# brown-palm/goal-force

Measured on AMD Instinct MI355X. Metric: frames_per_sec (81-frame video / (50-step denoise loop + VAE decode), Wan2.2-I2V-A14B 832x480x81f), higher is better.
Workload: dtype bf16

## Files before the change

### goal_force_amd/_lib.py

```python
from __future__ import annotations

import ctypes
import os
import threading

_HERE = os.path.dirname(os.path.abspath(__file__))
LIB_PATH = os.path.join(_HERE, "libgoalforce_hip.so")
LIB_PATH = os.environ.get("GOALFORCE_HIP_LIB", LIB_PATH)

SYMBOLS = (
    "gf_version", "gf_last_error", "gf_abi_version", "gf_set_option", "gf_get_option", "gf_reset_options",
    "gf_modulation", "gf_layernorm_modulate", "gf_rmsnorm_rope", "gf_gemm_bf16", "gf_flash_attn_fwd",
    "gf_patchify_im2col", "gf_unpatchify", "gf_cfg_euler_step", "gf_act", "gf_add_bf16",
    "gf_force_map",
    "gf_vae_prep_latent", "gf_vae_im2col", "gf_vae_finish_latent", "gf_vae_rmsnorm_silu", "gf_softmax_rows", "gf_rowmax_neg_bf16", "gf_transpose_pad",
    "gf_vae_tile_blend", "gf_vae_tile_finalize",
    "gf_quant_fp8_rowscale", "gf_cast_fp8", "gf_gemm_fp8", "gf_layernorm_modulate_fp8", "gf_modulate", "gf_gate_residual", "gf_rope_apply", "gf_linear_vt32_fp8",
    "gf_flash_attn_fwd_lse", "gf_flash_attn_bwd", "gf_flash_attn_bwd_workspace_bytes",
    "gf_layernorm_bwd", "gf_rmsnorm_rope_bwd", "gf_colsum", "gf_act_bwd", "gf_mse_loss", "gf_adamw_step", "gf_f32_to_bf16", "gf_sumsq",
    "gf_transpose_v", "gf_flash_attn_fwd_vt", "gf_transpose_v32", "gf_flash_attn_fwd_vt32", "gf_linear_vt32",
    "gf_conv3d_bf16", "gf_conv3d_padded_bf16", "gf_vae_rmsnorm_silu_padded", "gf_vae_upsample2x_padded", "gf_gemm_bf16_batched", "gf_transpose_pad_batched",
    "gf_resize_lanczos4_u8", "gf_resize_area_u8", "gf_canny_u8", "gf_flash_attn_fwd_lastmult",
)

ABI_VERSION = 18

EPI_BIAS, EPI_BIAS_GELU_TANH, EPI_BIAS_GATE_RESID, EPI_BIAS_RESID, EPI_BIAS_SILU, EPI_BIAS_MUL = range(6)


class GoalForceError(RuntimeError):
    """Raised when the HIP library is missing or a gf_* call returns an error."""


_lib = None
_lock = threading.Lock()

_vp, _i64, _f32, _int = ctypes.c_void_p, ctypes.c_int64, ctypes.c_float, ctypes.c_int


def _declare(lib):
    lib.gf_version.restype = ctypes.c_char_p
    lib.gf_version.argtypes = []
    lib.gf_last_error.restype = ctypes.c_char_p
    lib.gf_last_error.argtypes = []
    lib.gf_abi_version.restype = _int
    lib.gf_abi_version.argtypes = []
    lib.gf_set_option.restype = _int
    lib.gf_set_option.argtypes = [ctypes.c_char_p, _int]
    lib.gf_get_option.restype = _int
    lib.gf_get_option.argtypes = [ctypes.c_char_p, ctypes.POINTER(_int)]
    lib.gf_reset_options.restype = None
    lib.gf_reset_options.argtypes = []
    sigs = {
        "gf_layernorm_modulate": [_vp, _vp, _vp, _vp, _vp, _vp, _i64, _i64, _i64, _i64, _f32, _vp],
        "gf_modulation": [_vp, _vp, _vp, _i64, _i64, _i64, ctypes.c_uint32, _vp],
        "gf_rmsnorm_rope": [_vp, _vp, _vp, _vp, _i64, _i64, _i64, _i64, _f32, _vp],
        "gf_gemm_bf16": [_vp, _i64, _vp, _i64, _vp, _vp, _i64, _i64, _i64, _i64, _int, _vp, _i64, _vp, _vp],
        "gf_flash_attn_fwd": [_vp, _vp, _vp, _vp, _i64, _i64, _i64, _i64, _i64, _i64, _i64, _i64, _f32, _vp],
        "gf_flash_attn_fwd_lastmult": [_vp, _vp, _vp, _vp, _i64, _i64, _i64, _i64, _i64, _i64, _i64, _i64, _f32, _f32, _vp],
        "gf_flash_attn_fwd_lse": [_vp, _vp, _vp, _vp, _vp, _i64, _i64, _i64, _i64, _i64, _i64, _i64, _i64, _f32, _vp],
        "gf_flash_attn_bwd": [_vp] * 10 + [_i64] * 12 + [_f32, _vp],
        "gf_flash_attn_bwd_workspace_bytes": [_i64] * 3,
        "gf_layernorm_bwd": [_vp, _i64, _vp, _i64, _vp, _vp, _i64, _vp, _vp, _i64, _i64, _f32, _vp],
        "gf_rmsnorm_rope_bwd": [_vp, _i64, _vp, _i64, _vp, _vp, _vp, _vp, _i64, _vp, _i64, _i64, _i64, _f32, _vp],
        "gf_colsum": [_vp, _i64, _vp, _i64, _vp, _vp, _i64, _vp, _i64, _i64, _vp],
        "gf_act_bwd": [_vp, _vp, _vp, _i64, _int, _vp],
        "gf_mse_loss": [_vp, _vp, _vp, _vp, _i64, _f32, _vp],
        "gf_adamw_step": [_vp, _vp, _vp, _vp, _i64, _f32, _f32, _f32, _f32, _f32, _i64, _f32, _vp],
        "gf_f32_to_bf16": [_vp, _vp, _i64, _vp],
        "gf_sumsq": [_vp, _i64, _vp, _vp],
        "gf_transpose_v": [_vp, _i64, _vp, _i64, _i64, _i64, _vp],
        "gf_flash_attn_fwd_vt": [_vp, _vp, _vp, _vp, _vp, _i64, _i64, _i64, _i64, _i64, _i64, _i64, _i64, _f32, _vp],
        "gf_transpose_v32": [_vp, _i64, _vp, _i64, _i64, _i64, _vp],
        "gf_linear_vt32": [_vp, _i64, _vp, _i64, _vp, _vp, _i64, _i64, _i64, _i64, _vp],
        "gf_flash_attn_fwd_vt32": [_vp, _vp, _vp, _vp, _vp, _i64, _i64, _i64, _i64, _i64, _i64, _i64, _i64, _f32, _vp],
        "gf_patchify_im2col": [_vp, _i64, _vp, _i64, _vp, _i64, _i64, _i64, _i64, _vp],
        "gf_unpatchify": [_vp, _vp, _i64, _i64, _i64, _i64, _vp],
        "gf_cfg_euler_step": [_vp, _vp, _vp, _f32, _f32, _i64, _vp],
        "gf_act": [_vp, _vp, _i64, _int, _vp],
        "gf_add_bf16": [_vp, _vp, _vp, _i64, _vp],
        "gf_vae_prep_latent": [_vp, _i64, _i64, _i64, _i64, _vp, _vp, _vp, _i64, _i64, _i64, _i64, _i64, _vp],
        "gf_vae_im2col": [_vp, _vp, _vp, _i64, _i64, _i64, _i64, _i64, _i64, _int, _i64, _i64, _i64, _vp],
        "gf_conv3d_bf16": [_vp, _vp, _vp, _i64, _vp, _vp, _i64, _i64, _i64, _i64, _i64, _i64, _int, _int, _int, _int, _int,
                           _i64, _i64, _int, _vp, _i64, _vp],
        "gf_vae_finish_latent": [_vp, _i64, _vp, _vp, _vp, _i64, _i64, _vp],
        "gf_vae_rmsnorm_silu": [_vp, _vp, _vp, _i64, _i64, _int, _vp],
        "gf_vae_rmsnorm_silu_padded": [_vp, _vp, _vp, _i64, _i64, _i64, _i64, _int, _vp],
        "gf_conv3d_padded_bf16": [_vp, _vp, _i64, _vp, _vp, _i64, _i64, _i64, _i64, _i64, _i64, _i64, _int, _vp, _i64, _vp],
        "gf_vae_upsample2x_padded": [_vp, _vp, _i64, _i64, _i64, _i64, _vp],
        "gf_softmax_rows": [_vp, _i64, _vp, _i64, _vp, _i64, _i64, _i64, _i64, _f32, _vp],
        "gf_rowmax_neg_bf16": [_vp, _i64, _vp, _i64, _i64, _i64, _vp],
        "gf_transpose_pad": [_vp, _i64, _vp, _i64, _i64, _i64, _vp],
# ... 65 lines not shown
```

### goal_force_amd/csrc/gf_abi.hip

```cpp
#include "gf_common.h"
#include <cstdarg>
#include <cstdio>
#include <cstdlib>
#include <cstring>

#define GF_ABI_VERSION 18

static thread_local char g_err[512] = "";

void gf_set_error(const char* fmt, ...) {
    va_list ap;
    va_start(ap, fmt);
    vsnprintf(g_err, sizeof(g_err), fmt, ap);
    va_end(ap);
}

extern "C" GF_API const char* gf_version(void) { return "goalforce-hip 0.1.0 gfx950"; }
extern "C" GF_API const char* gf_last_error(void) { return g_err; }
extern "C" GF_API int gf_abi_version(void) { return GF_ABI_VERSION; }

static GfOptions g_options;

const GfOptions& gf_options() { return g_options; }

namespace {
struct OptionSlot {
    const char* name;
    std::atomic<int> GfOptions::*field;
    int lo, hi, dflt;
};
const OptionSlot kSlots[] = {
    {"prefer_8wave", &GfOptions::prefer_8wave, 0, 1, 0}, {"a4_stagger", &GfOptions::a4_stagger, 0, 1 << 20, 2},
    {"a4_group_m", &GfOptions::a4_group_m, 0, 64, 0},    {"conv_nb", &GfOptions::conv_nb, 0, 2, 0},
    {"conv_gather", &GfOptions::conv_gather, 0, 1, 0},   {"vae_rms3", &GfOptions::vae_rms3, 0, 1, 1},
    {"conv_direct", &GfOptions::conv_direct, 0, 1, 1},
};
}

extern "C" GF_API int gf_set_option(const char* name, int value) {
// ... 25 lines not shown
```

### goal_force_amd/dit.py

```python
from __future__ import annotations

import math
from typing import Optional, Tuple

import torch
import torch.nn as nn

from . import ops
from ._lib import GoalForceError


def precompute_freqs_cis(dim: int, end: int = 1024, theta: float = 10000.0):
    freqs = 1.0 / (theta ** (torch.arange(0, dim, 2)[: (dim // 2)].double() / dim))
    freqs = torch.outer(torch.arange(end), freqs)
    return torch.polar(torch.ones_like(freqs), freqs)


def precompute_freqs_cis_3d(dim: int, end: int = 1024, theta: float = 10000.0):
    return (precompute_freqs_cis(dim - 2 * (dim // 3), end, theta),
            precompute_freqs_cis(dim // 3, end, theta),
            precompute_freqs_cis(dim // 3, end, theta))


class RopeTable:
# ... 204 lines not shown
        x2 = _tokens2d(x)
        a = self.attend(x2, _as_rope(freqs, x.device))
        return linear(a, self.o).view(x.shape)


class CrossAttention(nn.Module):

    def __init__(self, dim: int, num_heads: int, eps: float = 1e-6, has_image_input: bool = False):
        super().__init__()
        if has_image_input:
            raise NotImplementedError("has_image_input=True (CLIP image tokens) is outside the Goal-Force path")
        self.dim, self.num_heads, self.head_dim = dim, num_heads, dim // num_heads
        self.q, self.k, self.v, self.o = (nn.Linear(dim, dim) for _ in range(4))
        self.norm_q, self.norm_k = RMSNorm(dim, eps=eps), RMSNorm(dim, eps=eps)
        self.has_image_input = False

    def context_kv(self, ctx2: torch.Tensor, fold: bool = True, pad_n: Optional[int] = None):
        m = 1
        if fold and ctx2.is_cuda and ops._OPT["fold_pad_keys"]:
            n = pad_run(ctx2) if pad_n is None else pad_n
            if ctx2.shape[0] - n >= 2 and n + 1 < ops.VT_MIN_KV:
                m = ctx2.shape[0] - n
                ctx2 = ctx2[: n + 1]
        cin = QuantizedInput(ctx2) if getattr(self.k, "_gf_w8", None) is not None else ctx2
        k, v = linear(cin, self.k), linear(cin, self.v)
        ops.rmsnorm_rope(k, self.norm_k.weight, None, None, self.head_dim, self.norm_k.eps)
        return k, v, m

    def attend(self, x2, kv):
        q = linear(x2, self.q)
        ops.rmsnorm_rope(q, self.norm_q.weight, None, None, self.head_dim, self.norm_q.eps)
        return ops.flash_attn(q, kv[0], kv[1], self.num_heads, last_key_mult=kv[2] if len(kv) > 2 else 1)

    def forward(self, x: torch.Tensor, y: torch.Tensor):
        x2 = _tokens2d(x)
        a = self.attend(x2, self.context_kv(_tokens2d(y)))
        return linear(a, self.o).view(x.shape)


class GateModule(nn.Module):

    def forward(self, x, gate, residual):
        if x.shape != residual.shape:
            raise GoalForceError("GateModule: x and residual must have the same shape")
        d = x.shape[-1]
        g = gate.reshape(-1, d)
        if x.dim() == 3 and g.shape[0] == x.shape[0] and x.shape[0] > 1:
            return torch.stack([ops.gate_residual(x[b], g[b].contiguous(), residual[b]) for b in range(x.shape[0])])
        if g.shape[0] != 1:
            raise GoalForceError("GateModule: gate must be [B or 1, 1, D] (per-token gates are outside the Goal-Force path)")
        return ops.gate_residual(x, g[0].contiguous(), residual)


class DiTBlock(nn.Module):

    def __init__(self, has_image_input: bool, dim: int, num_heads: int, ffn_dim: int, eps: float = 1e-6):
        super().__init__()
        self.dim, self.num_heads, self.ffn_dim, self.eps = dim, num_heads, ffn_dim, eps
        self.self_attn = SelfAttention(dim, num_heads, eps)
        self.cross_attn = CrossAttention(dim, num_heads, eps, has_image_input=has_image_input)
        self.norm1 = nn.LayerNorm(dim, eps=eps, elementwise_affine=False)
        self.norm2 = nn.LayerNorm(dim, eps=eps, elementwise_affine=False)
        self.norm3 = nn.LayerNorm(dim, eps=eps)
        self.ffn = nn.Sequential(nn.Linear(dim, ffn_dim), nn.GELU(approximate="tanh"), nn.Linear(ffn_dim, dim))
        self.modulation = nn.Parameter(torch.randn(1, 6, dim) / dim ** 0.5)
        self.gate = GateModule()
# ... 6 lines not shown
        rope = _as_rope(freqs, x.device)
        mod = ops.modulation(self.modulation, t_mod.contiguous(), onep_mask=0b010010)
        fp8 = getattr(self.ffn[0], "_gf_w8", None) is not None
        if self_attn_memo is not None and "x" in self_attn_memo:
            x_new = self_attn_memo.pop("x")
            ev = self_attn_memo.pop("ev", None)
            if ev is not None:
                torch.cuda.current_stream(x_new.device).wait_event(ev)
                x_new.record_stream(torch.cuda.current_stream(x_new.device))
            if out is not None:
                x_new = out.copy_(x_new)
            h = None if fp8 else torch.empty_like(x2)
        else:
            if fp8:
                h = QuantizedInput.layernorm(x2, scale1p=mod[1], shift=mod[0], eps=self.eps)
            else:
                h = ops.layernorm_modulate(x2, scale1p=mod[1], shift=mod[0], eps=self.eps)
            a = self.self_attn.attend(h, rope, sp, keep)
            x_new = out if out is not None else torch.empty_like(x2)
            linear(a, self.self_attn.o, epilogue=ops.EPI_BIAS_GATE_RESID, resid=x2, gate=mod[2], out=x_new)
            if keep is not None and keep.get("wide"):
                keep["x1"] = x_new.clone()
            if self_attn_memo is not None:
                self_attn_memo["x"] = x_new.clone()
                if x_new.is_cuda:
                    self_attn_memo["ev"] = torch.cuda.Event()
                    self_attn_memo["ev"].record(torch.cuda.current_stream(x_new.device))
        if fp8:
            h = QuantizedInput.layernorm(x_new, weight=self.norm3.weight, bias=self.norm3.bias, eps=self.eps)
        else:
            ops.layernorm_modulate(x_new, weight=self.norm3.weight, bias=self.norm3.bias, eps=self.eps, out=h)
        if context_kv is None:
            context_kv = self.cross_attn.context_kv(_tokens2d(context), fold=fold_pad_keys and keep is None, pad_n=pad_n)
        a = self.cross_attn.attend(h, context_kv)
        linear(a, self.cross_attn.o, epilogue=ops.EPI_BIAS_RESID, resid=x_new, out=x_new)
        if keep is not None and keep.get("wide"):
            keep["x2b"] = x_new.clone()
        if fp8:
            h = QuantizedInput.layernorm(x_new, scale1p=mod[4], shift=mod[3], eps=self.eps)
        else:
            ops.layernorm_modulate(x_new, scale1p=mod[4], shift=mod[3], eps=self.eps, out=h)
        f1 = linear(h, self.ffn[0], epilogue=ops.EPI_BIAS_GELU_TANH)
        linear(f1, self.ffn[2], epilogue=ops.EPI_BIAS_GATE_RESID, resid=x_new, gate=mod[5], out=x_new)
        return x_new.view(x.shape)


class Head(nn.Module):

    def __init__(self, dim: int, out_dim: int, patch_size: Tuple[int, int, int], eps: float):
        super().__init__()
        self.dim, self.patch_size, self.eps = dim, patch_size, eps
        self.norm = nn.LayerNorm(dim, eps=eps, elementwise_affine=False)
        self.head = nn.Linear(dim, out_dim * math.prod(patch_size))
        self.modulation = nn.Parameter(torch.randn(1, 2, dim) / dim ** 0.5)

    def forward(self, x, t_mod):
        if t_mod.dim() == 3:
            raise NotImplementedError("per-token head modulation is outside the Goal-Force path")
        x2 = _tokens2d(x)
        mod = ops.modulation(self.modulation, t_mod.contiguous(), onep_mask=0b10)
        h = ops.layernorm_modulate(x2, scale1p=mod[1], shift=mod[0], eps=self.eps)
        y = ops.gemm(h, self.head.weight, self.head.bias)
        return y.view(x.shape[:-1] + (y.shape[-1],))


class WanModel(nn.Module):

    def __init__(self, dim: int, in_dim: int, ffn_dim: int, out_dim: int, text_dim: int, freq_dim: int, eps: float,
# ... 101 lines not shown
```

### goal_force_amd/model_fn.py

```python
from __future__ import annotations

from typing import Optional

import torch

from . import ops
from ._lib import GoalForceError
from .dit import WanModel, pad_run


class ContextCache:

    def __init__(self):
        self.ctx = None
        self.pad_n = None
        self.dit_kv = {}
        self.cn_kv = {}


def _unsupported(name, value, default=None):
    if value is not None and value is not default and value is not False:
        raise NotImplementedError(f"model_fn_wan_video: `{name}` is outside the Goal-Force sampling path "
                                  "(SURVEY.md §2 #2)")


@torch.no_grad()
def model_fn_wan_video(
    dit: WanModel,
    motion_controller=None,
    vace=None,
    latents: torch.Tensor = None,
    timestep: torch.Tensor = None,
    context: torch.Tensor = None,
    clip_feature: Optional[torch.Tensor] = None,
    y: Optional[torch.Tensor] = None,
    reference_latents=None,
    vace_context=None,
    vace_scale=1.0,
    audio_embeds: Optional[torch.Tensor] = None,
    motion_latents: Optional[torch.Tensor] = None,
    s2v_pose_latents: Optional[torch.Tensor] = None,
    drop_motion_frames: bool = True,
    tea_cache=None,
    use_unified_sequence_parallel: bool = False,
    motion_bucket_id: Optional[torch.Tensor] = None,
    sliding_window_size: Optional[int] = None,
    sliding_window_stride: Optional[int] = None,
    cfg_merge: bool = False,
    use_gradient_checkpointing: bool = False,
    use_gradient_checkpointing_offload: bool = False,
# ... 29 lines not shown

    t, t_mod = dit.time_embed(timestep)

    if context_cache is not None and context_cache.ctx is not None:
        ctx, pad_n = context_cache.ctx, context_cache.pad_n
    else:
        ctx = dit.embed_text(context)
        pad_n = pad_run(ctx[0]) if ops._OPT["fold_pad_keys"] else None
        if context_cache is not None:
            context_cache.ctx, context_cache.pad_n = ctx, pad_n

    x, (f, h, w) = dit.patchify(latents, extra=y if (y is not None and dit.require_vae_embedding) else None)
    x = x[0]
    rope = dit.rope_table(f, h, w, latents.device)
    if sp is not None:
        x = sp.shard_tokens(x).contiguous()
        rope = dit.rope_table_shard(f, h, w, latents.device, sp)

    run_cn = use_controlnet and not (elide_zero_controlnet and controlnet.all_zero())
    c = None
    if run_cn:
        if controlnet.stride is not None:
            raise NotImplementedError("strided ControlNet (apply_strided_controlnet) is not used by Goal Force")
        control_latents = kwargs.get("control_signal_video_latents", None)
        if control_latents is None:
            raise GoalForceError("controlnet given but control_signal_video_latents missing")
        c = controlnet.controlnet_patch_embedding(control_latents)[0]
        if sp is not None:
            c = sp.shard_tokens(c).contiguous()
        n_cn = controlnet.controlnet_dit.num_layers
    else:
        n_cn = 0

    def kv_for(cache_dict, block, idx):
        if context_cache is None:
            return None
        if idx not in cache_dict:
            cache_dict[idx] = block.cross_attn.context_kv(ctx[0], pad_n=pad_n)
        return cache_dict[idx]

    for block_id, block in enumerate(dit.blocks):
        memo_cn = memo_dit = None
        if cfg_shared is not None and block_id == 0:
            memo_cn, memo_dit = cfg_shared.setdefault("cn0", {}), cfg_shared.setdefault("dit0", {})
        if block_id < n_cn:
            cb = controlnet.controlnet_dit.blocks[block_id]
            c = cb(c, ctx, t_mod, rope, context_kv=kv_for(context_cache.cn_kv if context_cache else None, cb, block_id),
                   sp=sp, self_attn_memo=memo_cn, pad_n=pad_n)
        x = block(x, ctx, t_mod, rope, context_kv=kv_for(context_cache.dit_kv if context_cache else None, block, block_id),
                  sp=sp, self_attn_memo=memo_dit, pad_n=pad_n)
        if block_id < n_cn:
            ops.gemm(c, controlnet.zero_conv_weight(block_id), controlnet.controlnet_zero_convs_after[block_id].bias,
                     epilogue=ops.EPI_BIAS_RESID, resid=x, out=x)

    x = dit.head(x.unsqueeze(0), t)
    if sp is not None:
        x = sp.gather_tokens(x[0], total=f * h * w).unsqueeze(0)
    return dit.unpatchify(x, (f, h, w))
```

### goal_force_amd/ops.py

```python
from __future__ import annotations

import math

import torch

from . import _lib
from ._lib import (EPI_BIAS, EPI_BIAS_GATE_RESID, EPI_BIAS_GELU_TANH, EPI_BIAS_MUL, EPI_BIAS_RESID, EPI_BIAS_SILU,
                   GoalForceError)

__all__ = [
    "modulation", "layernorm_modulate", "rmsnorm_rope", "gate_residual", "gemm", "flash_attn", "patchify_im2col", "unpatchify",
    "cfg_euler_step", "act", "add", "force_map",
    "EPI_BIAS", "EPI_BIAS_GELU_TANH", "EPI_BIAS_GATE_RESID", "EPI_BIAS_RESID", "EPI_BIAS_SILU", "EPI_BIAS_MUL",
]

_BF16 = torch.bfloat16

PROFILE_ATTN = None
PROFILE_GEMM = None
PROFILE_CONV = None


def _stream(t: torch.Tensor):
    if t.device.index != torch.cuda.current_device():
# ... 123 lines not shown
        out = torch.empty(a.shape[:-1] + (N,), dtype=_BF16, device=a.device)
    ov, Mo, No, ldc = _rows2d(out, "gemm.out")
    if (Mo, No) != (M, N):
        raise GoalForceError(f"gemm.out: expected [{M}, {N}], got [{Mo}, {No}]")
    ldr = 0
    if resid is not None:
        _req(resid, "gemm.resid")
        rv, Mr, Nr, ldr = _rows2d(resid, "gemm.resid")
        if (Mr, Nr) != (M, N):
            raise GoalForceError("gemm.resid: shape mismatch")
        resid = rv
    if gate is not None:
        _req(gate, "gemm.gate")
        if gate.numel() != N or not gate.is_contiguous():
            raise GoalForceError(f"gemm.gate: expected contiguous [{N}]")
    if bias is not None:
        _req(bias, "gemm.bias")
        if bias.numel() != N or not bias.is_contiguous():
            raise GoalForceError(f"gemm.bias: expected contiguous [{N}]")
    prof = PROFILE_GEMM
    if prof is not None:
        e0, e1 = torch.cuda.Event(enable_timing=True), torch.cuda.Event(enable_timing=True)
        e0.record()
    _lib.check(_lib.load().gf_gemm_bf16(_ptr(av), lda, _ptr(w), w.stride(0), _ptr(bias), _ptr(ov), ldc, M, N, K,
                                        int(epilogue), _ptr(resid), ldr, _ptr(gate), _stream(a)), "gf_gemm_bf16")
    if prof is not None:
        e1.record()
        prof.append((e0, e1, M, N, K, int(epilogue)))
    return out


VT_MIN_KV = 2048
_LIB_DEFAULTS = {"prefer_8wave": 0, "a4_stagger": 2, "a4_group_m": 0, "conv_nb": 0, "conv_gather": 0, "conv_direct": 1, "vae_rms3": 1}
_OPT = {"attn_k3": True, "vt_from_gemm": True, "conv_padded": True, "fold_pad_keys": True, "attn_q_prescale": True, "vae_attn_offset": True}


def lib_option(name: str) -> int:
    import ctypes
    v = ctypes.c_int(0)
    _lib.check(_lib.load().gf_get_option(name.encode(), ctypes.byref(v)), f"gf_get_option({name})")
    return int(v.value)


class options:

    def __init__(self, **kv):
        for k in kv:
            if k not in _OPT and k not in _LIB_DEFAULTS:
                raise GoalForceError(f"ops.options: unknown option {k!r}")
        self.kv, self.old = kv, {}

    @staticmethod
    def _apply_one(k, v):
        if k in _OPT:
            _OPT[k] = bool(v)
        else:
            _lib.check(_lib.load().gf_set_option(k.encode(), int(v)), f"gf_set_option({k})")

    def __enter__(self):
        self.old = {}
        try:
            for k, v in self.kv.items():
                old = _OPT[k] if k in _OPT else lib_option(k)
                self._apply_one(k, v)
                self.old[k] = old
        except BaseException:
            self.__exit__(None, None, None)
# ... 83 lines not shown
    if prof is not None:
        e0, e1 = torch.cuda.Event(enable_timing=True), torch.cuda.Event(enable_timing=True)
        e0.record()
    lib = _lib.load()
    kv_pad = -(-skv // 64) * 64
    if last_key_mult != 1 and (vt is not None or skv >= VT_MIN_KV):
        raise GoalForceError("flash_attn: last_key_mult is for short key sequences (the text context), not the V^T path")
    if skv >= VT_MIN_KV and head_dim == 128 and num_heads * 128 * kv_pad < 2 ** 31:
        if finished_q and vt is not None:
            raise GoalForceError("flash_attn: finished_q goes to kernel 2, which does not take kernel 3's V^T operand")
        k3 = _OPT["attn_k3"] and not finished_q
        tr, fa = (lib.gf_transpose_v32, lib.gf_flash_attn_fwd_vt32) if k3 else (lib.gf_transpose_v, lib.gf_flash_attn_fwd_vt)
        if vt is None:
            vt = _vt_workspace(num_heads * 128 * kv_pad, q.device)
            _lib.check(tr(_ptr(v), v.stride(0), _ptr(vt), skv, kv_pad, num_heads, _stream(q)), "gf_transpose_v")
        elif vt.numel() < num_heads * 128 * kv_pad:
            raise GoalForceError("flash_attn.vt: buffer smaller than heads*128*kv_pad")
        _lib.check(fa(_ptr(q), _ptr(k), _ptr(vt), _ptr(out), None, sq, skv, kv_pad, num_heads, head_dim,
                      q.stride(0), k.stride(0), out.stride(0), float(scale), _stream(q)), "gf_flash_attn_fwd_vt")
    elif last_key_mult != 1:
        _lib.check(lib.gf_flash_attn_fwd_lastmult(_ptr(q), _ptr(k), _ptr(v), _ptr(out), sq, skv, num_heads, head_dim, q.stride(0),
                                                  k.stride(0), v.stride(0), out.stride(0), float(scale), float(last_key_mult), _stream(q)),
                   "gf_flash_attn_fwd_lastmult")
    else:
        _lib.check(lib.gf_flash_attn_fwd(_ptr(q), _ptr(k), _ptr(v), _ptr(out), sq, skv, num_heads, head_dim,
                                         q.stride(0), k.stride(0), v.stride(0), out.stride(0), float(scale),
                                         _stream(q)), "gf_flash_attn_fwd")
    if prof is not None:
        e1.record()
        prof.append((e0, e1, sq, skv, num_heads))
    return out


def flash_attn_lse(q, k, v, num_heads, scale=None):
    for n, t in (("q", q), ("k", k), ("v", v)):
        _req(t, f"flash_attn_lse.{n}")
        if t.dim() != 2 or t.stride(1) != 1:
            raise GoalForceError(f"flash_attn_lse.{n}: expected 2-D [len, heads*head_dim] with contiguous rows")
    sq, hd_all = q.shape
    skv = k.shape[0]
    head_dim = hd_all // num_heads
    if k.shape[1] != hd_all or v.shape != k.shape or head_dim * num_heads != hd_all:
        raise GoalForceError("flash_attn_lse: q/k/v shape mismatch")
    if scale is None:
        scale = 1.0 / math.sqrt(head_dim)
    out = torch.empty((sq, hd_all), dtype=_BF16, device=q.device)
    lse = torch.empty((sq, num_heads), dtype=torch.float32, device=q.device)
    lib = _lib.load()
    kv_pad = -(-skv // 64) * 64
    if skv >= VT_MIN_KV and head_dim == 128 and num_heads * 128 * kv_pad < 2 ** 31:
        vt = _vt_workspace(num_heads * 128 * kv_pad, q.device)
        k3 = _OPT["attn_k3"]
        tr, fa = (lib.gf_transpose_v32, lib.gf_flash_attn_fwd_vt32) if k3 else (lib.gf_transpose_v, lib.gf_flash_attn_fwd_vt)
        _lib.check(tr(_ptr(v), v.stride(0), _ptr(vt), skv, kv_pad, num_heads, _stream(q)), "gf_transpose_v")
        _lib.check(fa(_ptr(q), _ptr(k), _ptr(vt), _ptr(out), _ptr(lse), sq, skv, kv_pad, num_heads, head_dim,
                      q.stride(0), k.stride(0), out.stride(0), float(scale), _stream(q)), "gf_flash_attn_fwd_vt")
        return out, lse
    _lib.check(lib.gf_flash_attn_fwd_lse(_ptr(q), _ptr(k), _ptr(v), _ptr(out), _ptr(lse), sq, skv, num_heads, head_dim,
                                         q.stride(0), k.stride(0), v.stride(0), out.stride(0), float(scale),
                                         _stream(q)), "gf_flash_attn_fwd_lse")
    return out, lse


def flash_attn_bwd(q, k, v, o, dout, lse, num_heads, scale=None, need_dkv=True):
    for n, t in (("q", q), ("k", k), ("v", v), ("o", o), ("dout", dout)):
        _req(t, f"flash_attn_bwd.{n}")
# ... 552 lines not shown
```

### include/goalforce.h

```cpp
#ifndef GOALFORCE_H
#define GOALFORCE_H

#include <stdint.h>

#if defined(GF_BUILD)
#define GF_API __attribute__((visibility("default")))
#else
#define GF_API
#endif

#ifdef __cplusplus
extern "C" {
#endif

typedef enum {
    GF_OK = 0,
    GF_ERR_INVALID_ARG = -1,
    GF_ERR_UNSUPPORTED = -2,
    GF_ERR_LAUNCH = -3
} gf_status;

GF_API const char* gf_version(void);
GF_API const char* gf_last_error(void);
GF_API int gf_abi_version(void);
// ... 21 lines not shown
    GF_EPI_BIAS_SILU = 4,
    GF_EPI_BIAS_MUL = 5
} gf_epilogue;

GF_API int gf_gemm_bf16(const void* A, int64_t lda, const void* W, int64_t ldw, const void* bias,
                 void* C, int64_t ldc, int64_t M, int64_t N, int64_t K,
                 int epilogue, const void* resid, int64_t ldr, const void* gate,
                 void* stream);

GF_API int gf_gemm_bf16_batched(const void* A, int64_t lda, int64_t strideA, const void* W, int64_t ldw, int64_t strideW, void* C,
                                int64_t ldc, int64_t strideC, int64_t M, int64_t N, int64_t K, int64_t batch, void* stream);

GF_API int gf_flash_attn_fwd(const void* q, const void* k, const void* v, void* o,
                      int64_t q_len, int64_t kv_len, int64_t heads, int64_t head_dim,
                      int64_t q_stride, int64_t k_stride, int64_t v_stride, int64_t o_stride,
                      float scale, void* stream);

GF_API int gf_transpose_v(const void* v, int64_t v_stride, void* vt, int64_t kv_len, int64_t kv_pad, int64_t heads, void* stream);
GF_API int gf_flash_attn_fwd_vt(const void* q, const void* k, const void* vt, void* o, float* lse,
                         int64_t q_len, int64_t kv_len, int64_t kv_pad, int64_t heads, int64_t head_dim,
                         int64_t q_stride, int64_t k_stride, int64_t o_stride, float scale, void* stream);

GF_API int gf_transpose_v32(const void* v, int64_t v_stride, void* vt, int64_t kv_len, int64_t kv_pad, int64_t heads, void* stream);
GF_API int gf_flash_attn_fwd_vt32(const void* q, const void* k, const void* vt, void* o, float* lse,
                                  int64_t q_len, int64_t kv_len, int64_t kv_pad, int64_t heads, int64_t head_dim,
                                  int64_t q_stride, int64_t k_stride, int64_t o_stride, float scale, void* stream);

GF_API int gf_linear_vt32(const void* x, int64_t ldx, const void* w, int64_t ldw, const void* bias, void* vt,
                          int64_t kv_len, int64_t kv_pad, int64_t N, int64_t K, void* stream);

GF_API int gf_flash_attn_fwd_lastmult(const void* q, const void* k, const void* v, void* o, int64_t q_len, int64_t kv_len,
                                      int64_t heads, int64_t head_dim, int64_t q_stride, int64_t k_stride, int64_t v_stride,
                                      int64_t o_stride, float scale, float last_key_multiplicity, void* stream);

GF_API int gf_flash_attn_fwd_lse(const void* q, const void* k, const void* v, void* o, float* lse,
                          int64_t q_len, int64_t kv_len, int64_t heads, int64_t head_dim,
                          int64_t q_stride, int64_t k_stride, int64_t v_stride, int64_t o_stride,
                          float scale, void* stream);
GF_API int64_t gf_flash_attn_bwd_workspace_bytes(int64_t q_len, int64_t kv_len, int64_t heads);
GF_API int gf_flash_attn_bwd(const void* q, const void* k, const void* v, const void* o, const void* dout,
                      const float* lse, void* workspace, void* dq, void* dk, void* dv,
                      int64_t q_len, int64_t kv_len, int64_t heads, int64_t head_dim,
                      int64_t q_stride, int64_t k_stride, int64_t v_stride, int64_t o_stride, int64_t do_stride,
                      int64_t dq_stride, int64_t dk_stride, int64_t dv_stride, float scale, void* stream);

GF_API int gf_layernorm_bwd(const void* x, int64_t x_stride, const void* dy, int64_t dy_stride, const void* g, void* dx,
                            int64_t dx_stride, float* dg_acc, float* db_acc, int64_t rows, int64_t dim, float eps, void* stream);
GF_API int gf_rmsnorm_rope_bwd(const void* x, int64_t x_stride, const void* dy, int64_t dy_stride, const void* weight,
                               const float* cos_tab, const float* sin_tab, void* dx, int64_t dx_stride, float* dw_acc,
                               int64_t rows, int64_t dim, int64_t head_dim, float eps, void* stream);
GF_API int gf_colsum(const void* a, int64_t lda, const void* b, int64_t ldb, const void* gate, void* out, int64_t ldo,
                     float* acc, int64_t rows, int64_t cols, void* stream);
GF_API int gf_act_bwd(const void* u, const void* df, void* du, int64_t n, int kind, void* stream);
GF_API int gf_mse_loss(const void* pred, const void* target, void* dpred, float* loss, int64_t n, float weight, void* stream);
GF_API int gf_adamw_step(void* param, const void* grad, float* exp_avg, float* exp_avg_sq, int64_t n, float lr, float beta1,
                         float beta2, float eps, float weight_decay, int64_t step, float grad_scale, void* stream);
GF_API int gf_f32_to_bf16(const float* src, void* dst, int64_t n, void* stream);
GF_API int gf_sumsq(const void* x, int64_t n, float* acc, void* stream);

GF_API int gf_patchify_im2col(const void* src0, int64_t c0, const void* src1, int64_t c1,
                       void* out, int64_t F, int64_t H, int64_t W, int64_t kpad, void* stream);

GF_API int gf_unpatchify(const void* tokens, void* out, int64_t c, int64_t f, int64_t h, int64_t w,
                  void* stream);

GF_API int gf_cfg_euler_step(void* latents, const void* posi, const void* nega,
// ... 93 lines not shown
```

Baseline: 0.6202.

## Fold cross-attention V and output projection into a cached per-head table

For cross-attention with few context keys (folded padding keys), the code now computes softmax probabilities per head with a dedicated kernel. It then multiplies them by a precomputed table U = V_h·W_o_h^T, replacing the flash-attention call plus the output-projection GEMM. U is cached per block in the context cache, so it is built once per run rather than per step. The output GEMM's K dimension shrinks from heads*128 to heads*n_pad, and a low-order correction term handles bf16 rounding of the last-key weight. The cost is extra memory for the cached tables, plus a different bf16 rounding path for the probabilities.

```diff
diff --git a/goal_force_amd/_lib.py b/goal_force_amd/_lib.py
--- a/goal_force_amd/_lib.py
+++ b/goal_force_amd/_lib.py
@@ -21,9 +21,10 @@
     "gf_transpose_v", "gf_flash_attn_fwd_vt", "gf_transpose_v32", "gf_flash_attn_fwd_vt32", "gf_linear_vt32",
     "gf_conv3d_bf16", "gf_conv3d_padded_bf16", "gf_vae_rmsnorm_silu_padded", "gf_vae_upsample2x_padded", "gf_gemm_bf16_batched", "gf_transpose_pad_batched",
     "gf_resize_lanczos4_u8", "gf_resize_area_u8", "gf_canny_u8", "gf_flash_attn_fwd_lastmult",
+    "gf_cross_probs", "gf_cross_fold_table",
 )
 
-ABI_VERSION = 18
+ABI_VERSION = 19
 
 EPI_BIAS, EPI_BIAS_GELU_TANH, EPI_BIAS_GATE_RESID, EPI_BIAS_RESID, EPI_BIAS_SILU, EPI_BIAS_MUL = range(6)
 
@@ -58,6 +59,8 @@
         "gf_gemm_bf16": [_vp, _i64, _vp, _i64, _vp, _vp, _i64, _i64, _i64, _i64, _int, _vp, _i64, _vp, _vp],
         "gf_flash_attn_fwd": [_vp, _vp, _vp, _vp, _i64, _i64, _i64, _i64, _i64, _i64, _i64, _i64, _f32, _vp],
         "gf_flash_attn_fwd_lastmult": [_vp, _vp, _vp, _vp, _i64, _i64, _i64, _i64, _i64, _i64, _i64, _i64, _f32, _f32, _vp],
+        "gf_cross_probs": [_vp, _vp, _vp, _i64, _i64, _i64, _i64, _i64, _i64, _i64, _i64, _f32, _f32, _vp],
+        "gf_cross_fold_table": [_vp, _vp, _vp, _i64, _i64, _i64, _i64, _i64, _i64, _i64, _i64, _vp],
         "gf_flash_attn_fwd_lse": [_vp, _vp, _vp, _vp, _vp, _i64, _i64, _i64, _i64, _i64, _i64, _i64, _i64, _f32, _vp],
         "gf_flash_attn_bwd": [_vp] * 10 + [_i64] * 12 + [_f32, _vp],
         "gf_flash_attn_bwd_workspace_bytes": [_i64] * 3,
diff --git a/goal_force_amd/csrc/gf_abi.hip b/goal_force_amd/csrc/gf_abi.hip
--- a/goal_force_amd/csrc/gf_abi.hip
+++ b/goal_force_amd/csrc/gf_abi.hip
@@ -4,7 +4,7 @@
 #include <cstdlib>
 #include <cstring>
 
-#define GF_ABI_VERSION 18
+#define GF_ABI_VERSION 19
 
 static thread_local char g_err[512] = "";
 
diff --git a/goal_force_amd/csrc/gf_cross_fold.hip b/goal_force_amd/csrc/gf_cross_fold.hip
--- /dev/null
+++ b/goal_force_amd/csrc/gf_cross_fold.hip
@@ -0,0 +1,206 @@
+#include "gf_common.h"
+
+namespace {
+
+constexpr int CF_HD = 128;
+constexpr int CF_MAXK = 64;
+constexpr int CF_THREADS = 256;
+constexpr int CF_QB = 128;
+
+__device__ __forceinline__ void cf_mfma32(f32x16& acc, const bf16x8& a, const bf16x8& b) {
+    acc = __builtin_amdgcn_mfma_f32_32x32x16_bf16(a, b, acc, 0, 0, 0);
+}
+
+__global__ __launch_bounds__(CF_THREADS) void cross_probs_kernel(const u16* __restrict__ q, const u16* __restrict__ k, u16* __restrict__ pout,
+                                                                 int q_len, int n_keys, int n_pad, int heads, long q_stride, long k_stride,
+                                                                 long p_stride, float c, float last_key_bias) {
+    __shared__ __attribute__((aligned(16))) char lds[CF_MAXK * 256];
+    const int tid = threadIdx.x;
+    const int lane = tid & 63, wave = tid >> 6;
+    const int r = lane & 31, h = lane >> 5;
+    const int head = blockIdx.y;
+    const int q0 = blockIdx.x * CF_QB + wave * 32;
+    const int halves = n_keys > 32 ? 2 : 1;
+
+#pragma unroll
+    for (int i = 0; i < (CF_MAXK * 16) / CF_THREADS; ++i) {
+        const int idx = tid + CF_THREADS * i;
+        const int row = idx >> 4, ch = idx & 15;
+        u16x8 v8 = {0, 0, 0, 0, 0, 0, 0, 0};
+        if (row < n_keys) v8 = *reinterpret_cast<const u16x8*>(k + (long)row * k_stride + head * CF_HD + ch * 8);
+        const int sk = ((row & 3) << 2) | ((row >> 2) & 3);
+        *(u16x8*)(lds + row * 256 + ((ch ^ sk) << 4)) = v8;
+    }
+
+    bf16x8 qf[8];
+    {
+        const int qr = min(q0 + r, q_len - 1);
+        const u16* qp = q + (long)qr * q_stride + head * CF_HD + 8 * h;
+#pragma unroll
+        for (int kd = 0; kd < 8; ++kd) qf[kd] = *reinterpret_cast<const bf16x8*>(qp + 16 * kd);
+    }
+    __syncthreads();
+
+    f32x16 sc[2];
+#pragma unroll
+    for (int e = 0; e < 16; ++e) {
+        sc[0][e] = 0.f;
+        sc[1][e] = 0.f;
+    }
+    const int sK = ((r & 3) << 2) | ((r >> 2) & 3);
+#pragma unroll
+    for (int kd = 0; kd < 8; ++kd) {
+        const int off = 256 * r + 16 * ((2 * kd + h) ^ sK);
+        cf_mfma32(sc[0], *(const bf16x8*)(lds + off), qf[kd]);
+        if (halves == 2) cf_mfma32(sc[1], *(const bf16x8*)(lds + off + 32 * 256), qf[kd]);
+    }
+
+#pragma unroll
+    for (int e = 0; e < 16; ++e) {
+        const int key = 4 * h + (e & 3) + 8 * (e >> 2);
+        if (key >= n_keys) sc[0][e] = -INFINITY;
+        if (key + 32 >= n_keys) sc[1][e] = -INFINITY;
+        if (key == n_keys - 1) sc[0][e] += last_key_bias;
+        if (key + 32 == n_keys - 1) sc[1][e] += last_key_bias;
+    }
+    float mx = sc[0][0];
+#pragma unroll
+    for (int e = 1; e < 16; ++e) mx = fmaxf(mx, sc[0][e]);
+#pragma unroll
+    for (int e = 0; e < 16; ++e) mx = fmaxf(mx, sc[1][e]);
+    mx = fmaxf(mx, __shfl_xor(mx, 32));
+    const float mc = mx * c;
+    float rs = 0.f;
+#pragma unroll
+    for (int e = 0; e < 16; ++e) {
+        sc[0][e] = __builtin_amdgcn_exp2f(__builtin_fmaf(sc[0][e], c, -mc));
+        sc[1][e] = __builtin_amdgcn_exp2f(__builtin_fmaf(sc[1][e], c, -mc));
+        rs += sc[0][e] + sc[1][e];
+    }
+    const float l_tot = rs + __shfl_xor(rs, 32);
+    const float inv = 1.0f / l_tot;
+    float pl = 0.f;
+#pragma unroll
+    for (int e = 0; e < 16; ++e) {
+        const int key = 4 * h + (e & 3) + 8 * (e >> 2);
+        if (key == n_keys - 1) pl = sc[0][e];
+        if (key + 32 == n_keys - 1) pl = sc[1][e];
+    }
+    pl += __shfl_xor(pl, 32);
+    const float wl = pl * inv;
+    const float wl_lo = wl - bf2f(f2bf(wl));
+
+    const int qrow = q0 + r;
+    if (qrow < q_len) {
+        u16* prow = pout + (long)qrow * p_stride + (long)head * n_pad;
+#pragma unroll
+        for (int half = 0; half < 2; ++half)
+#pragma unroll
+            for (int g = 0; g < 4; ++g) {
+                const int key = 32 * half + 8 * g + 4 * h;
+                if (key < n_pad) {
+                    float w4[4];
+#pragma unroll
+                    for (int i = 0; i < 4; ++i) w4[i] = key + i == n_keys ? wl_lo : sc[half][4 * g + i] * inv;
+                    u32x2 pk;
+                    pk[0] = pack2bf(w4[0], w4[1]);
+                    pk[1] = pack2bf(w4[2], w4[3]);
+                    *reinterpret_cast<u32x2*>(prow + key) = pk;
+                }
+            }
+    }
+}
+
+constexpr int CFT_ROWS = 64;
+__global__ __launch_bounds__(CF_THREADS) void cross_fold_table_kernel(const u16* __restrict__ v, const u16* __restrict__ w, u16* __restrict__ u,
+                                                                      int n_keys, int n_pad, int n_out, long v_stride, long w_stride,
+                                                                      long u_stride) {
+    __shared__ __attribute__((aligned(16))) u16 vs[CF_MAXK * CF_HD];
+    const int tid = threadIdx.x;
+    const int head = blockIdx.y;
+    for (int idx = tid; idx < n_pad * 16; idx += CF_THREADS) {
+        const int row = idx >> 4, ch = idx & 15;
+        u16x8 v8 = {0, 0, 0, 0, 0, 0, 0, 0};
+        if (row <= n_keys) v8 = *reinterpret_cast<const u16x8*>(v + (long)min(row, n_keys - 1) * v_stride + head * CF_HD + ch * 8);
+        *reinterpret_cast<u16x8*>(vs + row * CF_HD + ch * 8) = v8;
+    }
+    __syncthreads();
+    const int n = blockIdx.x * CFT_ROWS + (tid >> 2), jg = tid & 3;
+    if (n >= n_out) return;
+    const int nj = n_pad >> 2;
+    float acc[CF_MAXK / 4];
+#pragma unroll
+    for (int i = 0; i < CF_MAXK / 4; ++i) acc[i] = 0.f;
+    const u16* wr = w + (long)n * w_stride + head * CF_HD;
+    for (int d0 = 0; d0 < CF_HD; d0 += 8) {
+        const u16x8 w8 = *reinterpret_cast<const u16x8*>(wr + d0);
+        float wf[8];
+#pragma unroll
+        for (int e = 0; e < 8; ++e) wf[e] = bf2f(w8[e]);
+#pragma unroll
+        for (int i = 0; i < CF_MAXK / 4; ++i) {
+            if (i < nj) {
+                const u16x8 v8 = *reinterpret_cast<const u16x8*>(vs + (jg + 4 * i) * CF_HD + d0);
+#pragma unroll
+                for (int e = 0; e < 8; ++e) acc[i] = __builtin_fmaf(bf2f(v8[e]), wf[e], acc[i]);
+            }
+        }
+    }
+    u16* ur = u + (long)n * u_stride + (long)head * n_pad;
+#pragma unroll
+    for (int i = 0; i < CF_MAXK / 4; ++i) {
+        const int j = jg + 4 * i;
+        if (i < nj) ur[j] = j <= n_keys ? f2bf(acc[i]) : (u16)0;
+    }
+}
+
+}
+
+extern "C" GF_API int gf_cross_probs(const void* q, const void* k, void* p, int64_t q_len, int64_t n_keys, int64_t n_pad, int64_t heads,
+                                     int64_t head_dim, int64_t q_stride, int64_t k_stride, int64_t p_stride, float scale,
+                                     float last_key_multiplicity, void* stream) {
+    GF_CHECK_ARG(q && k && p, "gf_cross_probs: null pointer");
+    if (head_dim != CF_HD) {
+        gf_set_error("gf_cross_probs: head_dim=%ld unsupported (kernel is built for 128)", (long)head_dim);
+        return GF_ERR_UNSUPPORTED;
+    }
+    GF_CHECK_ARG(q_len >= 0 && q_len < (1 << 30) && heads > 0 && heads < 65536, "gf_cross_probs: bad sizes q=%ld heads=%ld", (long)q_len,
+                 (long)heads);
+    GF_CHECK_ARG(n_keys >= 1 && n_pad % 16 == 0 && n_pad > n_keys && n_pad <= CF_MAXK,
+                 "gf_cross_probs: 1 <= n_keys=%ld < n_pad=%ld <= 64, n_pad a multiple of 16", (long)n_keys, (long)n_pad);
+    GF_CHECK_ARG(q_stride % 8 == 0 && k_stride % 8 == 0 && p_stride % 4 == 0 && q_stride >= heads * CF_HD && k_stride >= heads * CF_HD &&
+                     p_stride >= heads * n_pad,
+                 "gf_cross_probs: strides must cover the rows (q, k: multiples of 8; p: of 4, >= heads * n_pad)");
+    GF_CHECK_ARG(gf_aligned16(q) && gf_aligned16(k) && ((uintptr_t)p & 7u) == 0, "gf_cross_probs: alignment (q, k 16 bytes, p 8 bytes)");
+    GF_CHECK_ARG(scale > 0.f && last_key_multiplicity >= 1.0f, "gf_cross_probs: scale > 0, multiplicity >= 1");
+    if (q_len == 0) return GF_OK;
+    const float c = scale * 1.4426950408889634f;
+    const float bias = last_key_multiplicity != 1.0f ? log2f(last_key_multiplicity) / c : 0.f;
+    const dim3 grid((unsigned)((q_len + CF_QB - 1) / CF_QB), (unsigned)heads);
+    hipLaunchKernelGGL(cross_probs_kernel, grid, dim3(CF_THREADS), 0, (hipStream_t)stream, (const u16*)q, (const u16*)k, (u16*)p,
+                       (int)q_len, (int)n_keys, (int)n_pad, (int)heads, (long)q_stride, (long)k_stride, (long)p_stride, c, bias);
+    GF_CHECK_LAUNCH("gf_cross_probs");
+    return GF_OK;
+}
+
+extern "C" GF_API int gf_cross_fold_table(const void* v, const void* w_o, void* u, int64_t n_keys, int64_t n_pad, int64_t heads,
+                                          int64_t head_dim, int64_t n_out, int64_t v_stride, int64_t w_stride, int64_t u_stride,
+                                          void* stream) {
+    GF_CHECK_ARG(v && w_o && u, "gf_cross_fold_table: null pointer");
+    if (head_dim != CF_HD) {
+        gf_set_error("gf_cross_fold_table: head_dim=%ld unsupported (kernel is built for 128)", (long)head_dim);
+        return GF_ERR_UNSUPPORTED;
+    }
+    GF_CHECK_ARG(heads > 0 && heads < 65536 && n_out > 0 && n_out < (1 << 30), "gf_cross_fold_table: bad sizes heads=%ld N=%ld", (long)heads,
+                 (long)n_out);
+    GF_CHECK_ARG(n_keys >= 1 && n_pad % 16 == 0 && n_pad > n_keys && n_pad <= CF_MAXK,
+                 "gf_cross_fold_table: 1 <= n_keys=%ld < n_pad=%ld <= 64, n_pad a multiple of 16", (long)n_keys, (long)n_pad);
+    GF_CHECK_ARG(v_stride % 8 == 0 && w_stride % 8 == 0 && v_stride >= heads * CF_HD && w_stride >= heads * CF_HD && u_stride >= heads * n_pad,
+                 "gf_cross_fold_table: strides must cover the rows (v, w_o: multiples of 8; u >= heads * n_pad)");
+    GF_CHECK_ARG(gf_aligned16(v) && gf_aligned16(w_o) && ((uintptr_t)u & 1u) == 0, "gf_cross_fold_table: alignment");
+    const dim3 grid((unsigned)((n_out + CFT_ROWS - 1) / CFT_ROWS), (unsigned)heads);
+    hipLaunchKernelGGL(cross_fold_table_kernel, grid, dim3(CF_THREADS), 0, (hipStream_t)stream, (const u16*)v, (const u16*)w_o, (u16*)u,
+                       (int)n_keys, (int)n_pad, (int)n_out, (long)v_stride, (long)w_stride, (long)u_stride);
+    GF_CHECK_LAUNCH("gf_cross_fold_table");
+    return GF_OK;
+}
diff --git a/goal_force_amd/dit.py b/goal_force_amd/dit.py
--- a/goal_force_amd/dit.py
+++ b/goal_force_amd/dit.py
@@ -260,6 +260,29 @@
         ops.rmsnorm_rope(q, self.norm_q.weight, None, None, self.head_dim, self.norm_q.eps)
         return ops.flash_attn(q, kv[0], kv[1], self.num_heads, last_key_mult=kv[2] if len(kv) > 2 else 1)
 
+    FOLD_K_MAX = 2560
+
+    def fold_ok(self, kv) -> bool:
+        if not ops._OPT["fold_cross_o"] or torch.is_grad_enabled() or len(kv) < 3 or kv[2] == 1 or self.head_dim != 128:
+            return False
+        if getattr(self.o, "_gf_w8", None) is not None:
+            return False
+        n = kv[0].shape[0]
+        k = self.num_heads * self.fold_pad(n)
+        return n <= ops.CROSS_FOLD_MAX_KEYS and k <= self.FOLD_K_MAX and k % 64 == 0
+
+    @staticmethod
+    def fold_pad(n_keys: int) -> int:
+        return -(-(n_keys + 1) // 16) * 16
+
+    def fold_table(self, kv):
+        return ops.cross_fold_table(kv[1], self.o.weight, self.num_heads, self.fold_pad(kv[0].shape[0]))
+
+    def attend_probs(self, x2, kv):
+        q = linear(x2, self.q)
+        ops.rmsnorm_rope(q, self.norm_q.weight, None, None, self.head_dim, self.norm_q.eps)
+        return ops.cross_probs(q, kv[0], self.num_heads, self.fold_pad(kv[0].shape[0]), last_key_mult=kv[2])
+
     def forward(self, x: torch.Tensor, y: torch.Tensor):
         x2 = _tokens2d(x)
         a = self.attend(x2, self.context_kv(_tokens2d(y)))
@@ -332,8 +355,13 @@
             ops.layernorm_modulate(x_new, weight=self.norm3.weight, bias=self.norm3.bias, eps=self.eps, out=h)
         if context_kv is None:
             context_kv = self.cross_attn.context_kv(_tokens2d(context), fold=fold_pad_keys and keep is None, pad_n=pad_n)
-        a = self.cross_attn.attend(h, context_kv)
-        linear(a, self.cross_attn.o, epilogue=ops.EPI_BIAS_RESID, resid=x_new, out=x_new)
+        ca = self.cross_attn
+        if keep is None and not fp8 and ca.fold_ok(context_kv):
+            u = context_kv[3] if len(context_kv) > 3 else ca.fold_table(context_kv)
+            ops.gemm(ca.attend_probs(h, context_kv), u, ca.o.bias, epilogue=ops.EPI_BIAS_RESID, resid=x_new, out=x_new)
+        else:
+            a = ca.attend(h, context_kv)
+            linear(a, ca.o, epilogue=ops.EPI_BIAS_RESID, resid=x_new, out=x_new)
         if keep is not None and keep.get("wide"):
             keep["x2b"] = x_new.clone()
         if fp8:
diff --git a/goal_force_amd/model_fn.py b/goal_force_amd/model_fn.py
--- a/goal_force_amd/model_fn.py
+++ b/goal_force_amd/model_fn.py
@@ -16,6 +16,8 @@
         self.pad_n = None
         self.dit_kv = {}
         self.cn_kv = {}
+        self.dit_u = {}
+        self.cn_u = {}
 
 
 def _unsupported(name, value, default=None):
@@ -111,12 +113,17 @@
     else:
         n_cn = 0
 
-    def kv_for(cache_dict, block, idx):
+    def kv_for(cache_dict, u_dict, block, idx):
         if context_cache is None:
             return None
         if idx not in cache_dict:
             cache_dict[idx] = block.cross_attn.context_kv(ctx[0], pad_n=pad_n)
-        return cache_dict[idx]
+        kv = cache_dict[idx]
+        if block.cross_attn.fold_ok(kv):
+            if idx not in u_dict:
+                u_dict[idx] = block.cross_attn.fold_table(kv)
+            kv = kv + (u_dict[idx],)
+        return kv
 
     for block_id, block in enumerate(dit.blocks):
         memo_cn = memo_dit = None
@@ -124,9 +131,11 @@
             memo_cn, memo_dit = cfg_shared.setdefault("cn0", {}), cfg_shared.setdefault("dit0", {})
         if block_id < n_cn:
             cb = controlnet.controlnet_dit.blocks[block_id]
-            c = cb(c, ctx, t_mod, rope, context_kv=kv_for(context_cache.cn_kv if context_cache else None, cb, block_id),
+            c = cb(c, ctx, t_mod, rope, context_kv=kv_for(context_cache.cn_kv if context_cache else None,
+                                                          context_cache.cn_u if context_cache else None, cb, block_id),
                    sp=sp, self_attn_memo=memo_cn, pad_n=pad_n)
-        x = block(x, ctx, t_mod, rope, context_kv=kv_for(context_cache.dit_kv if context_cache else None, block, block_id),
+        x = block(x, ctx, t_mod, rope, context_kv=kv_for(context_cache.dit_kv if context_cache else None,
+                                                         context_cache.dit_u if context_cache else None, block, block_id),
                   sp=sp, self_attn_memo=memo_dit, pad_n=pad_n)
         if block_id < n_cn:
             ops.gemm(c, controlnet.zero_conv_weight(block_id), controlnet.controlnet_zero_convs_after[block_id].bias,
diff --git a/goal_force_amd/ops.py b/goal_force_amd/ops.py
--- a/goal_force_amd/ops.py
+++ b/goal_force_amd/ops.py
@@ -179,7 +179,8 @@
 
 VT_MIN_KV = 2048
 _LIB_DEFAULTS = {"prefer_8wave": 0, "a4_stagger": 2, "a4_group_m": 0, "conv_nb": 0, "conv_gather": 0, "conv_direct": 1, "vae_rms3": 1}
-_OPT = {"attn_k3": True, "vt_from_gemm": True, "conv_padded": True, "fold_pad_keys": True, "attn_q_prescale": True, "vae_attn_offset": True}
+_OPT = {"attn_k3": True, "vt_from_gemm": True, "conv_padded": True, "fold_pad_keys": True, "attn_q_prescale": True, "vae_attn_offset": True,
+        "fold_cross_o": True}
 
 
 def lib_option(name: str) -> int:
@@ -329,6 +330,45 @@
     return out
 
 
+CROSS_FOLD_MAX_KEYS = 63
+
+
+def cross_probs(q, k, num_heads, n_pad, last_key_mult=1, scale=None, out=None):
+    for n, t in (("q", q), ("k", k)):
+        _req(t, f"cross_probs.{n}")
+        if t.dim() != 2 or t.stride(1) != 1:
+            raise GoalForceError(f"cross_probs.{n}: expected 2-D [len, heads*head_dim] with contiguous rows")
+    sq, hd_all = q.shape
+    n_keys = k.shape[0]
+    head_dim = hd_all // num_heads
+    if k.shape[1] != hd_all or head_dim * num_heads != hd_all:
+        raise GoalForceError("cross_probs: q/k shape mismatch")
+    if out is None:
+        out = torch.empty((sq, num_heads * n_pad), dtype=_BF16, device=q.device)
+    elif out.dtype != _BF16 or out.dim() != 2 or out.stride(1) != 1 or tuple(out.shape) != (sq, num_heads * n_pad):
+        raise GoalForceError(f"cross_probs.out: expected [{sq}, {num_heads * n_pad}] bf16 with contiguous rows")
+    if scale is None:
+        scale = 1.0 / math.sqrt(head_dim)
+    _lib.check(_lib.load().gf_cross_probs(_ptr(q), _ptr(k), _ptr(out), sq, n_keys, n_pad, num_heads, head_dim, q.stride(0), k.stride(0),
+                                          out.stride(0), float(scale), float(last_key_mult), _stream(q)), "gf_cross_probs")
+    return out
+
+
+def cross_fold_table(v, w_o, num_heads, n_pad):
+    for n, t in (("v", v), ("w_o", w_o)):
+        _req(t, f"cross_fold_table.{n}")
+        if t.dim() != 2 or t.stride(1) != 1:
+            raise GoalForceError(f"cross_fold_table.{n}: expected 2-D with contiguous rows")
+    n_keys, hd_all = v.shape
+    if w_o.shape[1] != hd_all or hd_all % num_heads:
+        raise GoalForceError("cross_fold_table: v / w_o shape mismatch")
+    N = w_o.shape[0]
+    u = torch.empty((N, num_heads * n_pad), dtype=_BF16, device=v.device)
+    _lib.check(_lib.load().gf_cross_fold_table(_ptr(v), _ptr(w_o), _ptr(u), n_keys, n_pad, num_heads, hd_all // num_heads, N, v.stride(0),
+                                               w_o.stride(0), u.stride(0), _stream(v)), "gf_cross_fold_table")
+    return u
+
+
 def flash_attn_lse(q, k, v, num_heads, scale=None):
     for n, t in (("q", q), ("k", k), ("v", v)):
         _req(t, f"flash_attn_lse.{n}")
diff --git a/include/goalforce.h b/include/goalforce.h
--- a/include/goalforce.h
+++ b/include/goalforce.h
@@ -77,6 +77,13 @@
 GF_API int gf_flash_attn_fwd_lastmult(const void* q, const void* k, const void* v, void* o, int64_t q_len, int64_t kv_len,
                                       int64_t heads, int64_t head_dim, int64_t q_stride, int64_t k_stride, int64_t v_stride,
                                       int64_t o_stride, float scale, float last_key_multiplicity, void* stream);
+
+GF_API int gf_cross_probs(const void* q, const void* k, void* p, int64_t q_len, int64_t n_keys, int64_t n_pad, int64_t heads,
+                          int64_t head_dim, int64_t q_stride, int64_t k_stride, int64_t p_stride, float scale,
+                          float last_key_multiplicity, void* stream);
+
+GF_API int gf_cross_fold_table(const void* v, const void* w_o, void* u, int64_t n_keys, int64_t n_pad, int64_t heads, int64_t head_dim,
+                               int64_t n_out, int64_t v_stride, int64_t w_stride, int64_t u_stride, void* stream);
 
 GF_API int gf_flash_attn_fwd_lse(const void* q, const void* k, const void* v, void* o, float* lse,
                           int64_t q_len, int64_t kv_len, int64_t heads, int64_t head_dim,
```

After: 0.6345, median of 6. 1.02x the previous value.
